# nii-yamagishilab/self-attention-tacotron

Hardware: AMD Instinct MI355X
Metric: mel-frames/sec (teacher-forced train step) (higher is better)
Workload: dtype bf16

## Files before the change

self-attention-tacotron_amd/csrc/flash.hip:

```cpp
#include <algorithm>
#include "common.h"

namespace {

constexpr int FHD = 128, FT = 64, FNT = 256;
constexpr float FLOG2E = 1.4426950408889634f;
typedef __attribute__((ext_vector_type(4))) unsigned int fu32x4_t;

__device__ __forceinline__ int kswz(int c) { return ((c & 3) << 1) ^ ((c >> 2) & 1); }

struct RowRegs { float4 v0[4], v1[4]; };
struct ColRegs { float4 v[2][4]; };
__device__ __forceinline__ void load_rows(const float* __restrict__ src, int64_t ld, int nvalid, int tid, RowRegs& R) {
#pragma unroll
  for (int g = 0; g < 4; ++g) {
    const int e = tid + FNT * g, row = min(e >> 4, nvalid - 1), chunk = e & 15;
    const float4* p = reinterpret_cast<const float4*>(src + (int64_t)row * ld + chunk * 8);
    R.v0[g] = p[0]; R.v1[g] = p[1];
  }
}
__device__ __forceinline__ void store_rows(const RowRegs& R, int nvalid, uint16_t* __restrict__ dst, int tid) {
#pragma unroll
  for (int g = 0; g < 4; ++g) {
    const int e = tid + FNT * g, row = e >> 4, chunk = e & 15;
    fu32x4_t w;
    w[0] = pack_bf16x2(R.v0[g].x, R.v0[g].y); w[1] = pack_bf16x2(R.v0[g].z, R.v0[g].w);
    w[2] = pack_bf16x2(R.v1[g].x, R.v1[g].y); w[3] = pack_bf16x2(R.v1[g].z, R.v1[g].w);
    if (row >= nvalid) w = (fu32x4_t){0u, 0u, 0u, 0u};
    *reinterpret_cast<fu32x4_t*>(dst + (chunk * FT + (row ^ kswz(chunk & 7))) * 8) = w;
  }
}
__device__ __forceinline__ void load_cols(const float* __restrict__ src, int64_t ld, int nvalid, int tid, ColRegs& R) {
  const int cq = tid & 31;
#pragma unroll
  for (int pass = 0; pass < 2; ++pass) {
    const int rq = (tid >> 5) + 8 * pass;
#pragma unroll
    for (int r = 0; r < 4; ++r)
      R.v[pass][r] = *reinterpret_cast<const float4*>(src + (int64_t)min(4 * rq + r, nvalid - 1) * ld + 4 * cq);
  }
}
__device__ __forceinline__ void store_cols(const ColRegs& R, int nvalid, uint16_t* __restrict__ dst, int tid) {
  const int cq = tid & 31;
  const int pc0 = (cq >> 4) * 64 + (cq & 15);
#pragma unroll
  for (int pass = 0; pass < 2; ++pass) {
    const int rq = (tid >> 5) + 8 * pass;
    const int ks = rq >> 3, q8 = rq & 7, eh = q8 >> 2, g = q8 & 3;
    float f[16];
#pragma unroll
    for (int r = 0; r < 4; ++r) {
      const bool ok = 4 * rq + r < nvalid;
      const float4 v = R.v[pass][r];
      f[4 * r] = ok ? v.x : 0.f; f[4 * r + 1] = ok ? v.y : 0.f; f[4 * r + 2] = ok ? v.z : 0.f; f[4 * r + 3] = ok ? v.w : 0.f;
    }
#pragma unroll
    for (int ii = 0; ii < 4; ++ii) {
      uint2 w;
      w.x = pack_bf16x2(f[ii], f[4 + ii]); w.y = pack_bf16x2(f[8 + ii], f[12 + ii]);
      *reinterpret_cast<uint2*>(dst + (((ks * 4 + g) * FHD + pc0 + 16 * ii) * 8) + 4 * eh) = w;
    }
  }
}
__device__ __forceinline__ bf16x8_t frag_rows(const uint16_t* img, int t, int ks, int lane) {
  const int chunk = 4 * ks + (lane >> 4), row = 16 * t + (lane & 15);
  return *reinterpret_cast<const bf16x8_t*>(img + (chunk * FT + (row ^ kswz(chunk & 7))) * 8);
}
__device__ __forceinline__ bf16x8_t frag_cols(const uint16_t* img, int n, int ks, int lane) {
  return *reinterpret_cast<const bf16x8_t*>(img + ((ks * 4 + (lane >> 4)) * FHD + 16 * n + (lane & 15)) * 8);
}
__device__ __forceinline__ bf16x8_t frag_global(const float* __restrict__ rowp, bool valid, int ks, int lane) {
  const float4* p = reinterpret_cast<const float4*>(rowp + 32 * ks + 8 * (lane >> 4));
  const float4 v0 = p[0], v1 = p[1];
  fu32x4_t w;
  w[0] = pack_bf16x2(v0.x, v0.y); w[1] = pack_bf16x2(v0.z, v0.w);
  w[2] = pack_bf16x2(v1.x, v1.y); w[3] = pack_bf16x2(v1.z, v1.w);
  if (!valid) w = (fu32x4_t){0u, 0u, 0u, 0u};
  return __builtin_bit_cast(bf16x8_t, w);
}
__device__ __forceinline__ bf16x8_t pack_b(const f32x4_t& lo, const f32x4_t& hi) {
  fu32x4_t w;
  w[0] = pack_bf16x2(lo[0], lo[1]); w[1] = pack_bf16x2(lo[2], lo[3]);
  w[2] = pack_bf16x2(hi[0], hi[1]); w[3] = pack_bf16x2(hi[2], hi[3]);
  return __builtin_bit_cast(bf16x8_t, w);
}
__device__ __forceinline__ float col_max(float v, int lane) {
  v = fmaxf(v, swz_xor(v, 16));
  return fmaxf(v, __int_as_float(__builtin_amdgcn_ds_bpermute((lane ^ 32) << 2, __float_as_int(v))));
}
__device__ __forceinline__ float col_sum(float v, int lane) {
  v += swz_xor(v, 16);
  return v + __int_as_float(__builtin_amdgcn_ds_bpermute((lane ^ 32) << 2, __float_as_int(v)));
}
__device__ __forceinline__ int unperm(int pr) { return (pr & ~63) | ((pr & 15) << 2) | ((pr & 63) >> 4); }

struct RowRegsB { fu32x4_t v[4]; };
struct ColRegsB { uint2 v[2][4]; };
__device__ __forceinline__ void load_rows(const uint16_t* __restrict__ src, int64_t ld, int nvalid, int tid, RowRegsB& R) {
#pragma unroll
  for (int g = 0; g < 4; ++g) {
    const int e = tid + FNT * g, row = min(e >> 4, nvalid - 1), chunk = e & 15;
    R.v[g] = *reinterpret_cast<const fu32x4_t*>(src + (int64_t)row * ld + chunk * 8);
  }
}
__device__ __forceinline__ void store_rows(const RowRegsB& R, int nvalid, uint16_t* __restrict__ dst, int tid) {
#pragma unroll
  for (int g = 0; g < 4; ++g) {
    const int e = tid + FNT * g, row = e >> 4, chunk = e & 15;
    fu32x4_t w = R.v[g];
    if (row >= nvalid) w = (fu32x4_t){0u, 0u, 0u, 0u};
    *reinterpret_cast<fu32x4_t*>(dst + (chunk * FT + (row ^ kswz(chunk & 7))) * 8) = w;
  }
}
__device__ __forceinline__ void load_cols(const uint16_t* __restrict__ src, int64_t ld, int nvalid, int tid, ColRegsB& R) {
  const int cq = tid & 31;
#pragma unroll
  for (int pass = 0; pass < 2; ++pass) {
    const int rq = (tid >> 5) + 8 * pass;
#pragma unroll
    for (int r = 0; r < 4; ++r)
      R.v[pass][r] = *reinterpret_cast<const uint2*>(src + (int64_t)min(4 * rq + r, nvalid - 1) * ld + 4 * cq);
  }
}
__device__ __forceinline__ void store_cols(const ColRegsB& R, int nvalid, uint16_t* __restrict__ dst, int tid) {
  const int cq = tid & 31;
  const int pc0 = (cq >> 4) * 64 + (cq & 15);
#pragma unroll
  for (int pass = 0; pass < 2; ++pass) {
    const int rq = (tid >> 5) + 8 * pass;
    const int ks = rq >> 3, q8 = rq & 7, eh = q8 >> 2, g = q8 & 3;
    uint32_t lo[4], hi[4];
#pragma unroll
    for (int r = 0; r < 4; ++r) {
      const bool ok = 4 * rq + r < nvalid;
      lo[r] = ok ? R.v[pass][r].x : 0u; hi[r] = ok ? R.v[pass][r].y : 0u;
    }
#pragma unroll
    for (int ii = 0; ii < 4; ++ii) {
      const uint32_t* w4 = (ii >> 1) ? hi : lo;
      uint2 w;
      if (ii & 1) { w.x = (w4[0] >> 16) | (w4[1] & 0xFFFF0000u); w.y = (w4[2] >> 16) | (w4[3] & 0xFFFF0000u); }
      else { w.x = (w4[0] & 0xFFFFu) | (w4[1] << 16); w.y = (w4[2] & 0xFFFFu) | (w4[3] << 16); }
      *reinterpret_cast<uint2*>(dst + (((ks * 4 + g) * FHD + pc0 + 16 * ii) * 8) + 4 * eh) = w;
    }
  }
}
__device__ __forceinline__ bf16x8_t frag_global(const uint16_t* __restrict__ rowp, bool valid, int ks, int lane) {
  fu32x4_t w = *reinterpret_cast<const fu32x4_t*>(rowp + 32 * ks + 8 * (lane >> 4));
  if (!valid) w = (fu32x4_t){0u, 0u, 0u, 0u};
  return __builtin_bit_cast(bf16x8_t, w);
}
template <bool BF> struct FSrc { typedef float T; typedef RowRegs Row; typedef ColRegs Col; };
template <> struct FSrc<true> { typedef uint16_t T; typedef RowRegsB Row; typedef ColRegsB Col; };

struct FlashArgs {
  const float* k; const float* v; const float* q; int64_t ld;
  float* o; int64_t ldo; float* lse;
  const float* dout; const float* delta;
  float* dk; float* dv; float* dq; int64_t ldd;
  int T, H, B; float scale; int causal;
  const uint16_t* kb; const uint16_t* vb; const uint16_t* qb; int64_t ldb;
  const uint16_t* doutb; int64_t ldob;
  uint16_t* kb_out; uint16_t* vb_out; uint16_t* qb_out;
  int tile_lo, tile_n;
  uint32_t thresh; float dscale; uint32_t stream; const uint32_t* seed;
};

__device__ __forceinline__ void flash_block(int nt, int BH, int& tile, int& bh, int lin = (int)blockIdx.x) {
  if ((BH & 7) == 0) { const int slot = lin >> 3; bh = (slot / nt) * 8 + (lin & 7); tile = slot - (slot / nt) * nt; }
  else { bh = lin / nt; tile = lin - bh * nt; }
}

template <bool DROP>
__attribute__((amdgpu_waves_per_eu(2, 2)))
__global__ __launch_bounds__(FNT) void flash_fwd_k(const FlashArgs a) {
  __shared__ __attribute__((aligned(16))) uint16_t lds[2 * FT * FHD];
  uint16_t* Ks = lds;
  uint16_t* Vt = lds + FT * FHD;
  const int tid = threadIdx.x, lane = tid & 63, wave = tid >> 6, g = lane >> 4;
  const int T = a.T, nqt = (T + FT - 1) / FT;
  int bx, bh; flash_block(nqt, a.B * a.H, bx, bh);
  const int b = bh / a.H, h = bh - b * a.H;
  const int qt = nqt - 1 - bx, i0 = qt * FT;
  const float* K = a.k + (int64_t)b * T * a.ld + h * FHD;
  const float* V = a.v + (int64_t)b * T * a.ld + h * FHD;
  const float* Q = a.q + (int64_t)b * T * a.ld + h * FHD;
  const int iq = i0 + 16 * wave + (lane & 15);
  bf16x8_t qb[4];
#pragma unroll
  for (int ks = 0; ks < 4; ++ks) qb[ks] = frag_global(Q + (int64_t)min(iq, T - 1) * a.ld, iq < T, ks, lane);
  if (a.qb_out && iq < T) {
    uint16_t* qo = a.qb_out + ((int64_t)b * T + iq) * a.ldb + h * FHD;
#pragma unroll
    for (int ks = 0; ks < 4; ++ks) *reinterpret_cast<bf16x8_t*>(qo + 32 * ks + 8 * g) = qb[ks];
  }
  const uint32_t seed = (a.thresh && a.seed) ? *a.seed : 0u;
  const float c2 = a.scale * FLOG2E;
  float m = -INFINITY, lsum = 0.f;
  f32x4_t oacc[8];
#pragma unroll
  for (int n = 0; n < 8; ++n) oacc[n] = (f32x4_t){0.f, 0.f, 0.f, 0.f};
  const int nkt = a.causal ? qt + 1 : nqt;
  RowRegs rk; ColRegs rv;
  load_rows(K, a.ld, T, tid, rk);
  load_cols(V, a.ld, T, tid, rv);
  for (int kt = 0; kt < nkt; ++kt) {
    const int j0 = kt * FT;
    lds_barrier();
    store_rows(rk, T - j0, Ks, tid);
    store_cols(rv, T - j0, Vt, tid);
    if (a.kb_out && kt == qt) {
#pragma unroll
      for (int gq = 0; gq < 4; ++gq) {
        const int e = tid + FNT * gq, row = e >> 4, chunk = e & 15;
        if (j0 + row < T) {
          fu32x4_t w;
          w[0] = pack_bf16x2(rk.v0[gq].x, rk.v0[gq].y); w[1] = pack_bf16x2(rk.v0[gq].z, rk.v0[gq].w);
          w[2] = pack_bf16x2(rk.v1[gq].x, rk.v1[gq].y); w[3] = pack_bf16x2(rk.v1[gq].z, rk.v1[gq].w);
          *reinterpret_cast<fu32x4_t*>(a.kb_out + ((int64_t)b * T + j0 + row) * a.ldb + h * FHD + chunk * 8) = w;
        }
      }
      const int cq = tid & 31;
#pragma unroll
      for (int pass = 0; pass < 2; ++pass)
#pragma unroll
        for (int r = 0; r < 4; ++r) {
          const int row = 4 * ((tid >> 5) + 8 * pass) + r;
          if (j0 + row < T) {
            const float4 v = rv.v[pass][r];
            uint2 w; w.x = pack_bf16x2(v.x, v.y); w.y = pack_bf16x2(v.z, v.w);
            *reinterpret_cast<uint2*>(a.vb_out + ((int64_t)b * T + j0 + row) * a.ldb + h * FHD + 4 * cq) = w;
          }
        }
    }
    if (kt + 1 < nkt) {
      load_rows(K + (int64_t)(j0 + FT) * a.ld, a.ld, T - j0 - FT, tid, rk);
      load_cols(V + (int64_t)(j0 + FT) * a.ld, a.ld, T - j0 - FT, tid, rv);
    }
    lds_barrier();
    f32x4_t s[4];
#pragma unroll
    for (int j = 0; j < 4; ++j) {
      s[j] = (f32x4_t){0.f, 0.f, 0.f, 0.f};
#pragma unroll
      for (int ks = 0; ks < 4; ++ks) s[j] = __builtin_amdgcn_mfma_f32_16x16x32_bf16(frag_rows(Ks, j, ks, lane), qb[ks], s[j], 0, 0, 0);
    }
    float mx = -INFINITY;
#pragma unroll
    for (int j = 0; j < 4; ++j)
#pragma unroll
      for (int r = 0; r < 4; ++r) {
        const int key = j0 + 16 * j + 4 * g + r;
        const bool ok = (key < T) & (!a.causal | (key <= iq));
        s[j][r] = ok ? s[j][r] * c2 : -INFINITY;
        mx = fmaxf(mx, s[j][r]);
      }
    mx = col_max(mx, lane);
    const float mn = fmaxf(m, mx);
    const float alpha = exp2f_(m - mn);
    float rs = 0.f;
#pragma unroll
    for (int j = 0; j < 4; ++j)
#pragma unroll
      for (int r = 0; r < 4; ++r) {
        const float pv = exp2f_(s[j][r] - mn);
        rs += pv;
        float pd = pv;
        if constexpr (DROP) {
          const int key = j0 + 16 * j + 4 * g + r;
          pd = satt_keep(seed, a.stream, (uint32_t)(((int64_t)bh * T + iq) * T + key), a.thresh) ? pv * a.dscale : 0.f;
        }
        s[j][r] = pd;
      }
    rs = col_sum(rs, lane);
    lsum = lsum * alpha + rs;
    m = mn;
#pragma unroll
    for (int n = 0; n < 8; ++n)
#pragma unroll
      for (int r = 0; r < 4; ++r) oacc[n][r] *= alpha;
#pragma unroll
    for (int ks = 0; ks < 2; ++ks) {
      const bf16x8_t pb = pack_b(s[2 * ks], s[2 * ks + 1]);
#pragma unroll
      for (int n = 0; n < 8; ++n) oacc[n] = __builtin_amdgcn_mfma_f32_16x16x32_bf16(frag_cols(Vt, n, ks, lane), pb, oacc[n], 0, 0, 0);
    }
  }
  if (iq < T) {
    const float inv = 1.f / lsum;
    float* orow = a.o + ((int64_t)b * T + iq) * a.ldo + h * FHD;
#pragma unroll
    for (int bq = 0; bq < 2; ++bq)
#pragma unroll
      for (int r = 0; r < 4; ++r) {
        const float4 v = make_float4(oacc[4 * bq][r] * inv, oacc[4 * bq + 1][r] * inv, oacc[4 * bq + 2][r] * inv, oacc[4 * bq + 3][r] * inv);
        *reinterpret_cast<float4*>(orow + 64 * bq + 16 * g + 4 * r) = v;
      }
    if (g == 0) a.lse[(int64_t)bh * T + iq] = m + log2f(lsum);
  }
}

__global__ __launch_bounds__(256) void flash_delta_k(const float* __restrict__ o, const float* __restrict__ dout, int64_t ldo,
                                                     float* __restrict__ delta, int B, int T, int H,
                                                     uint16_t* __restrict__ doutb, int64_t ldob, int r0, int r1) {
  const int lane = threadIdx.x & 63;
  const int64_t w = blockIdx.x * 4 + (threadIdx.x >> 6);
  const int nr = r1 - r0;
  if (w >= (int64_t)B * nr * H) return;
  const int64_t rr = w / H; const int h = (int)(w - rr * H);
  const int64_t row = (rr / nr) * T + r0 + (rr % nr);
  const float2 x = *reinterpret_cast<const float2*>(o + row * ldo + h * FHD + 2 * lane);
  const float2 y = *reinterpret_cast<const float2*>(dout + row * ldo + h * FHD + 2 * lane);
  if (doutb) *reinterpret_cast<uint32_t*>(doutb + row * ldob + h * FHD + 2 * lane) = pack_bf16x2(y.x, y.y);
  const float s = wave_sum(x.x * y.x + x.y * y.y);
  if (lane == 0) { const int64_t b = row / T; delta[(b * H + h) * T + (row - b * T)] = s; }
}

constexpr int DKV_LDS = (4 * FT * FHD) * 2 + 2 * FT * 4;
template <bool BF, bool DROP>
__device__ __forceinline__ void flash_dkv_body(const FlashArgs& a, uint16_t* dyn, int lin) {
  typedef typename FSrc<BF>::T ST;
  const int64_t sld = BF ? a.ldb : a.ld, dld = BF ? a.ldob : a.ldo;
  uint16_t* Qs = dyn; uint16_t* Qt = dyn + FT * FHD; uint16_t* Ds = dyn + 2 * FT * FHD; uint16_t* Dt = dyn + 3 * FT * FHD;
  float* Ls = reinterpret_cast<float*>(dyn + 4 * FT * FHD); float* dl = Ls + FT;
  const int tid = threadIdx.x, lane = tid & 63, wave = tid >> 6, g = lane >> 4;
  const int T = a.T, nt = (T + FT - 1) / FT;
  int kt, bh; flash_block(a.tile_n, a.B * a.H, kt, bh, lin);
  kt += a.tile_lo;
  const int b = bh / a.H, h = bh - b * a.H;
  const int j0 = kt * FT;
  const ST* K = (BF ? (const ST*)a.kb : (const ST*)a.k) + (int64_t)b * T * sld + h * FHD;
  const ST* V = (BF ? (const ST*)a.vb : (const ST*)a.v) + (int64_t)b * T * sld + h * FHD;
  const ST* Q = (BF ? (const ST*)a.qb : (const ST*)a.q) + (int64_t)b * T * sld + h * FHD;
  const ST* DO = (BF ? (const ST*)a.doutb : (const ST*)a.dout) + (int64_t)b * T * dld + h * FHD;
  const int key = j0 + 16 * wave + (lane & 15);
  bf16x8_t kb[4], vb[4];
#pragma unroll
  for (int ks = 0; ks < 4; ++ks) {
    kb[ks] = frag_global(K + (int64_t)min(key, T - 1) * sld, key < T, ks, lane);
    vb[ks] = frag_global(V + (int64_t)min(key, T - 1) * sld, key < T, ks, lane);
  }
  const uint32_t seed = (a.thresh && a.seed) ? *a.seed : 0u;
  const float c2 = a.scale * FLOG2E;
  f32x4_t dvt[8], dkt[8];
#pragma unroll
  for (int n = 0; n < 8; ++n) { dvt[n] = (f32x4_t){0.f, 0.f, 0.f, 0.f}; dkt[n] = dvt[n]; }
  struct Stage { typename FSrc<BF>::Row rq, rd; typename FSrc<BF>::Col cq, cd; float rl, rdl; };
  constexpr int NS = BF ? 2 : 1;
  Stage st[NS];
  auto request = [&](Stage& S, int i0) {
    load_rows(Q + (int64_t)i0 * sld, sld, T - i0, tid, S.rq);
    load_cols(Q + (int64_t)i0 * sld, sld, T - i0, tid, S.cq);
    load_rows(DO + (int64_t)i0 * dld, dld, T - i0, tid, S.rd);
    load_cols(DO + (int64_t)i0 * dld, dld, T - i0, tid, S.cd);
    const int64_t li = (int64_t)bh * T + min(i0 + (tid & (FT - 1)), T - 1);
    S.rl = a.lse[li]; S.rdl = a.delta[li];
  };
  const int qt0 = a.causal ? kt : 0;
  auto step = [&](Stage& S, int qt) {
    const int i0 = qt * FT;
    lds_barrier();
    store_rows(S.rq, T - i0, Qs, tid);
    store_cols(S.cq, T - i0, Qt, tid);
    store_rows(S.rd, T - i0, Ds, tid);
    store_cols(S.cd, T - i0, Dt, tid);
    if (tid < FT) {
      const bool ok = i0 + tid < T;
      Ls[tid] = ok ? S.rl : 0.f;
      dl[tid] = ok ? S.rdl : 0.f;
    }
    if (qt + NS < nt) request(S, i0 + NS * FT);
    lds_barrier();
    f32x4_t pd[4], ds[4];
#pragma unroll
    for (int i = 0; i < 4; ++i) {
      f32x4_t s = (f32x4_t){0.f, 0.f, 0.f, 0.f}, dp = s;
#pragma unroll
      for (int ks = 0; ks < 4; ++ks) {
        s = __builtin_amdgcn_mfma_f32_16x16x32_bf16(frag_rows(Qs, i, ks, lane), kb[ks], s, 0, 0, 0);
        dp = __builtin_amdgcn_mfma_f32_16x16x32_bf16(frag_rows(Ds, i, ks, lane), vb[ks], dp, 0, 0, 0);
      }
#pragma unroll
      for (int r = 0; r < 4; ++r) {
        const int ql = 16 * i + 4 * g + r, q = i0 + ql;
        const bool ok = (q < T) & (key < T) & (!a.causal | (key <= q));
        const float ev = exp2f_(s[r] * c2 - Ls[ql]);
        const float pv = ok ? ev : 0.f;
        if constexpr (DROP) {
          const bool keep = satt_keep(seed, a.stream, (uint32_t)(((int64_t)bh * T + q) * T + key), a.thresh);
          pd[i][r] = keep ? pv * a.dscale : 0.f;
          ds[i][r] = pv * ((keep ? dp[r] * a.dscale : 0.f) - dl[ql]);
        } else {
          pd[i][r] = pv;
          ds[i][r] = pv * (dp[r] - dl[ql]);
        }
      }
    }
#pragma unroll
    for (int ks = 0; ks < 2; ++ks) {
      const bf16x8_t pb = pack_b(pd[2 * ks], pd[2 * ks + 1]), sb = pack_b(ds[2 * ks], ds[2 * ks + 1]);
#pragma unroll
      for (int n = 0; n < 8; ++n) {
        dvt[n] = __builtin_amdgcn_mfma_f32_16x16x32_bf16(frag_cols(Dt, n, ks, lane), pb, dvt[n], 0, 0, 0);
        dkt[n] = __builtin_amdgcn_mfma_f32_16x16x32_bf16(frag_cols(Qt, n, ks, lane), sb, dkt[n], 0, 0, 0);
      }
    }
  };
  request(st[0], qt0 * FT);
  if (NS == 2 && qt0 + 1 < nt) request(st[NS - 1], (qt0 + 1) * FT);
  for (int qt = qt0; qt < nt; qt += NS) {
    step(st[0], qt);
    if (NS == 2 && qt + 1 < nt) step(st[NS - 1], qt + 1);
  }
  if (key < T) {
    float* dkr = a.dk + ((int64_t)b * T + key) * a.ldd + h * FHD;
    float* dvr = a.dv + ((int64_t)b * T + key) * a.ldd + h * FHD;
#pragma unroll
    for (int bq = 0; bq < 2; ++bq)
#pragma unroll
      for (int r = 0; r < 4; ++r) {
        const int col = 64 * bq + 16 * g + 4 * r;
        *reinterpret_cast<float4*>(dvr + col) = make_float4(dvt[4 * bq][r], dvt[4 * bq + 1][r], dvt[4 * bq + 2][r], dvt[4 * bq + 3][r]);
        *reinterpret_cast<float4*>(dkr + col) = make_float4(dkt[4 * bq][r] * a.scale, dkt[4 * bq + 1][r] * a.scale,
                                                             dkt[4 * bq + 2][r] * a.scale, dkt[4 * bq + 3][r] * a.scale);
      }
  }
}

template <bool BF, bool DROP>
__device__ __forceinline__ void flash_dq_body(const FlashArgs& a, uint16_t* lds, int lin) {
  typedef typename FSrc<BF>::T ST;
  const int64_t sld = BF ? a.ldb : a.ld, dld = BF ? a.ldob : a.ldo;
  uint16_t* Ks = lds; uint16_t* Kt = lds + FT * FHD; uint16_t* Vs = lds + 2 * FT * FHD;
  const int tid = threadIdx.x, lane = tid & 63, wave = tid >> 6, g = lane >> 4;
  const int T = a.T;
  int bx, bh; flash_block(a.tile_n, a.B * a.H, bx, bh, lin);
  const int b = bh / a.H, h = bh - b * a.H;
  const int qt = a.tile_lo + a.tile_n - 1 - bx, i0 = qt * FT;
  const ST* K = (BF ? (const ST*)a.kb : (const ST*)a.k) + (int64_t)b * T * sld + h * FHD;
  const ST* V = (BF ? (const ST*)a.vb : (const ST*)a.v) + (int64_t)b * T * sld + h * FHD;
  const ST* Q = (BF ? (const ST*)a.qb : (const ST*)a.q) + (int64_t)b * T * sld + h * FHD;
  const ST* DO = (BF ? (const ST*)a.doutb : (const ST*)a.dout) + (int64_t)b * T * dld + h * FHD;
  const int iq = i0 + 16 * wave + (lane & 15);
  bf16x8_t qb[4], dob[4];
#pragma unroll
  for (int ks = 0; ks < 4; ++ks) {
    qb[ks] = frag_global(Q + (int64_t)min(iq, T - 1) * sld, iq < T, ks, lane);
    dob[ks] = frag_global(DO + (int64_t)min(iq, T - 1) * dld, iq < T, ks, lane);
  }
  const float Lq_ = a.lse[(int64_t)bh * T + min(iq, T - 1)], dqr_ = a.delta[(int64_t)bh * T + min(iq, T - 1)];
  const float Lq = iq < T ? Lq_ : 0.f, dq_ = iq < T ? dqr_ : 0.f;
  const uint32_t seed = (a.thresh && a.seed) ? *a.seed : 0u;
  const float c2 = a.scale * FLOG2E;
  f32x4_t dqt[8];
#pragma unroll
  for (int n = 0; n < 8; ++n) dqt[n] = (f32x4_t){0.f, 0.f, 0.f, 0.f};
  const int nkt = a.causal ? qt + 1 : (T + FT - 1) / FT;
  struct Stage { typename FSrc<BF>::Row rk, rv; typename FSrc<BF>::Col ck; };
  constexpr int NS = BF ? 2 : 1;
  Stage st[NS];
  auto request = [&](Stage& S, int j0) {
    load_rows(K + (int64_t)j0 * sld, sld, T - j0, tid, S.rk);
    load_cols(K + (int64_t)j0 * sld, sld, T - j0, tid, S.ck);
    load_rows(V + (int64_t)j0 * sld, sld, T - j0, tid, S.rv);
  };
  auto step = [&](Stage& S, int kt) {
    const int j0 = kt * FT;
    lds_barrier();
    store_rows(S.rk, T - j0, Ks, tid);
    store_cols(S.ck, T - j0, Kt, tid);
    store_rows(S.rv, T - j0, Vs, tid);
    if (kt + NS < nkt) request(S, j0 + NS * FT);
    lds_barrier();
    f32x4_t ds[4];
#pragma unroll
    for (int j = 0; j < 4; ++j) {
      f32x4_t s = (f32x4_t){0.f, 0.f, 0.f, 0.f}, dp = s;
#pragma unroll
      for (int ks = 0; ks < 4; ++ks) {
        s = __builtin_amdgcn_mfma_f32_16x16x32_bf16(frag_rows(Ks, j, ks, lane), qb[ks], s, 0, 0, 0);
        dp = __builtin_amdgcn_mfma_f32_16x16x32_bf16(frag_rows(Vs, j, ks, lane), dob[ks], dp, 0, 0, 0);
      }
#pragma unroll
      for (int r = 0; r < 4; ++r) {
        const int key = j0 + 16 * j + 4 * g + r;
        const bool ok = (iq < T) & (key < T) & (!a.causal | (key <= iq));
        const float ev = exp2f_(s[r] * c2 - Lq);
        const float pv = ok ? ev : 0.f;
        float dpr = dp[r];
        if constexpr (DROP)
          dpr = satt_keep(seed, a.stream, (uint32_t)(((int64_t)bh * T + iq) * T + key), a.thresh) ? dpr * a.dscale : 0.f;
        ds[j][r] = pv * (dpr - dq_);
      }
    }
#pragma unroll
    for (int ks = 0; ks < 2; ++ks) {
      const bf16x8_t sb = pack_b(ds[2 * ks], ds[2 * ks + 1]);
#pragma unroll
      for (int n = 0; n < 8; ++n) dqt[n] = __builtin_amdgcn_mfma_f32_16x16x32_bf16(frag_cols(Kt, n, ks, lane), sb, dqt[n], 0, 0, 0);
    }
  };
  request(st[0], 0);
  if (NS == 2 && 1 < nkt) request(st[NS - 1], FT);
  for (int kt = 0; kt < nkt; kt += NS) {
    step(st[0], kt);
    if (NS == 2 && kt + 1 < nkt) step(st[NS - 1], kt + 1);
  }
  if (iq < T) {
    float* dqr = a.dq + ((int64_t)b * T + iq) * a.ldd + h * FHD;
#pragma unroll
    for (int bq = 0; bq < 2; ++bq)
#pragma unroll
      for (int r = 0; r < 4; ++r)
        *reinterpret_cast<float4*>(dqr + 64 * bq + 16 * g + 4 * r) =
            make_float4(dqt[4 * bq][r] * a.scale, dqt[4 * bq + 1][r] * a.scale, dqt[4 * bq + 2][r] * a.scale, dqt[4 * bq + 3][r] * a.scale);
  }
}

inline bool fl16(const void* p) { return (reinterpret_cast<uintptr_t>(p) & 15) == 0; }

}

template <bool BF, bool DROP>
__global__ __launch_bounds__(FNT) void flash_bwd_k(const FlashArgs a, const int ntiles) {
  extern __shared__ __attribute__((aligned(16))) uint16_t dyn[];
  const int lin = (int)blockIdx.x;
  if (lin < ntiles) flash_dkv_body<BF, DROP>(a, dyn, lin);
  else flash_dq_body<BF, DROP>(a, dyn, lin - ntiles);
}

static int flash_fwd_launch(const float* k, const float* v, const float* q, int64_t ld, float* o, int64_t ldo, float* lse,
                            int B, int T, int H, int head_dim, float scale, int causal, uint32_t drop_thresh,
                            float drop_scale, uint32_t drop_stream, const uint32_t* seed, uint16_t* kb, uint16_t* vb,
                            uint16_t* qb, int64_t ldb, void* stream) {
  if (!k || !v || !q || !o || !lse || B <= 0 || T <= 0 || H <= 0) return SATT_E_BADARG;
  if (head_dim != FHD) return SATT_E_UNSUPPORTED;
  if (ld % 4 || ldo % 4 || !fl16(k) || !fl16(v) || !fl16(q) || !fl16(o)) return SATT_E_UNSUPPORTED;
  if ((int64_t)B * H > 65535 || (int64_t)B * H * T * T >= (1ll << 32)) return SATT_E_UNSUPPORTED;
  if (kb && (!vb || !qb || ldb % 8 || !fl16(kb) || !fl16(vb) || !fl16(qb))) return SATT_E_BADARG;
  FlashArgs a{};
  a.k = k; a.v = v; a.q = q; a.ld = ld; a.o = o; a.ldo = ldo; a.lse = lse; a.T = T; a.H = H; a.B = B; a.scale = scale; a.causal = causal;
  a.thresh = drop_thresh; a.dscale = drop_scale; a.stream = drop_stream; a.seed = seed;
  a.kb_out = kb; a.vb_out = vb; a.qb_out = qb; a.ldb = ldb;
  if (drop_thresh) hipLaunchKernelGGL(flash_fwd_k<true>, dim3(((T + FT - 1) / FT) * B * H), dim3(FNT), 0, (hipStream_t)stream, a);
  else hipLaunchKernelGGL(flash_fwd_k<false>, dim3(((T + FT - 1) / FT) * B * H), dim3(FNT), 0, (hipStream_t)stream, a);
  SATT_LAUNCH_CHECK();
  return SATT_OK;
}

extern "C" int satt_flash_attn_fwd(const float* k, const float* v, const float* q, int64_t ld, float* o, int64_t ldo, float* lse,
                                   int B, int T, int H, int head_dim, float scale, int causal, uint32_t drop_thresh,
                                   float drop_scale, uint32_t drop_stream, const uint32_t* seed, void* stream) {
  return flash_fwd_launch(k, v, q, ld, o, ldo, lse, B, T, H, head_dim, scale, causal, drop_thresh, drop_scale, drop_stream, seed,
                          nullptr, nullptr, nullptr, 0, stream);
}

extern "C" int satt_flash_attn_fwd_b(const float* k, const float* v, const float* q, int64_t ld, float* o, int64_t ldo, float* lse,
                                     int B, int T, int H, int head_dim, float scale, int causal, uint32_t drop_thresh,
                                     float drop_scale, uint32_t drop_stream, const uint32_t* seed, uint16_t* kb, uint16_t* vb,
                                     uint16_t* qb, int64_t ldb, void* stream) {
  if (!kb) return SATT_E_BADARG;
  return flash_fwd_launch(k, v, q, ld, o, ldo, lse, B, T, H, head_dim, scale, causal, drop_thresh, drop_scale, drop_stream, seed,
                          kb, vb, qb, ldb, stream);
}

static int flash_bwd_launch(const float* k, const float* v, const float* q, int64_t ld, const float* o, const float* dout,
                            int64_t ldo, const float* lse, float* delta, float* dk, float* dv, float* dq, int64_t ldd,
                            int B, int T, int H, int head_dim, float scale, int causal, uint32_t drop_thresh,
                            float drop_scale, uint32_t drop_stream, const uint32_t* seed, int tile_lo, int tile_hi,
                            int with_delta, const uint16_t* kb, const uint16_t* vb, const uint16_t* qb, int64_t ldb,
                            uint16_t* doutb, int64_t ldob, void* stream) {
  const bool bf = kb != nullptr;
  if ((!bf && (!k || !v || !q)) || !o || !dout || !lse || !delta || !dk || !dv || !dq || B <= 0 || T <= 0 || H <= 0) return SATT_E_BADARG;
  if (head_dim != FHD) return SATT_E_UNSUPPORTED;
  if (ldo % 4 || ldd % 4 || !fl16(o) || !fl16(dout) || !fl16(dk) || !fl16(dv) || !fl16(dq)) return SATT_E_UNSUPPORTED;
  if (!bf && (ld % 4 || !fl16(k) || !fl16(v) || !fl16(q))) return SATT_E_UNSUPPORTED;
  if (bf && (!vb || !qb || !doutb || ldb % 8 || ldob % 8 || !fl16(kb) || !fl16(vb) || !fl16(qb) || !fl16(doutb))) return SATT_E_BADARG;
  if ((int64_t)B * H > 65535 || (int64_t)B * H * T * T >= (1ll << 32)) return SATT_E_UNSUPPORTED;
  const int nt = (T + FT - 1) / FT;
  if (tile_lo < 0 || tile_hi > nt || tile_lo >= tile_hi) return SATT_E_BADARG;
  if (!causal && (tile_lo != 0 || tile_hi != nt)) return SATT_E_BADARG;
  FlashArgs a{};
  a.k = k; a.v = v; a.q = q; a.ld = ld; a.ldo = ldo; a.lse = const_cast<float*>(lse); a.dout = dout; a.delta = delta;
  a.dk = dk; a.dv = dv; a.dq = dq; a.ldd = ldd; a.T = T; a.H = H; a.B = B; a.scale = scale; a.causal = causal;
  a.tile_lo = tile_lo; a.tile_n = tile_hi - tile_lo;
  a.thresh = drop_thresh; a.dscale = drop_scale; a.stream = drop_stream; a.seed = seed;
  a.kb = kb; a.vb = vb; a.qb = qb; a.ldb = ldb; a.doutb = doutb; a.ldob = ldob;
  hipStream_t s = (hipStream_t)stream;
  const int r0 = tile_lo * FT, r1 = std::min(tile_hi * FT, T);
  const int64_t nw = (int64_t)B * (r1 - r0) * H;
  if (with_delta)
    hipLaunchKernelGGL(flash_delta_k, dim3((unsigned)((nw + 3) / 4)), dim3(256), 0, s, o, dout, ldo, delta, B, T, H,
                       bf ? doutb : (uint16_t*)nullptr, ldob, r0, r1);
  static_assert(DKV_LDS >= 3 * FT * FHD * 2, "the dQ body fits the dK/dV body's LDS");
  const int ntiles = a.tile_n * B * H;
#define SATT_FLASH_BWD(BFV, DRV)                                                                                        \
  do {                                                                                                                    \
    (void)hipFuncSetAttribute((const void*)flash_bwd_k<BFV, DRV>, hipFuncAttributeMaxDynamicSharedMemorySize, DKV_LDS);   \
    hipLaunchKernelGGL((flash_bwd_k<BFV, DRV>), dim3(2 * ntiles), dim3(FNT), DKV_LDS, s, a, ntiles);                      \
  } while (0)
  if (bf) { if (drop_thresh) SATT_FLASH_BWD(true, true); else SATT_FLASH_BWD(true, false); }
  else { if (drop_thresh) SATT_FLASH_BWD(false, true); else SATT_FLASH_BWD(false, false); }
#undef SATT_FLASH_BWD
  SATT_LAUNCH_CHECK();
  return SATT_OK;
}

extern "C" int satt_flash_attn_bwd_tiles(const float* k, const float* v, const float* q, int64_t ld, const float* o, const float* dout,
                                         int64_t ldo, const float* lse, float* delta, float* dk, float* dv, float* dq, int64_t ldd,
                                         int B, int T, int H, int head_dim, float scale, int causal, uint32_t drop_thresh,
                                         float drop_scale, uint32_t drop_stream, const uint32_t* seed, int tile_lo, int tile_hi,
                                         int with_delta, void* stream) {
  return flash_bwd_launch(k, v, q, ld, o, dout, ldo, lse, delta, dk, dv, dq, ldd, B, T, H, head_dim, scale, causal, drop_thresh,
                          drop_scale, drop_stream, seed, tile_lo, tile_hi, with_delta, nullptr, nullptr, nullptr, 0, nullptr, 0, stream);
}

extern "C" int satt_flash_attn_bwd_tiles_b(const uint16_t* kb, const uint16_t* vb, const uint16_t* qb, int64_t ldb, const float* o,
                                           const float* dout, int64_t ldo, uint16_t* doutb, int64_t ldob, const float* lse,
                                           float* delta, float* dk, float* dv, float* dq, int64_t ldd, int B, int T, int H,
                                           int head_dim, float scale, int causal, uint32_t drop_thresh, float drop_scale,
                                           uint32_t drop_stream, const uint32_t* seed, int tile_lo, int tile_hi, int with_delta,
                                           void* stream) {
  if (!kb) return SATT_E_BADARG;
  return flash_bwd_launch(nullptr, nullptr, nullptr, 0, o, dout, ldo, lse, delta, dk, dv, dq, ldd, B, T, H, head_dim, scale, causal,
                          drop_thresh, drop_scale, drop_stream, seed, tile_lo, tile_hi, with_delta, kb, vb, qb, ldb, doutb, ldob, stream);
}

extern "C" int satt_flash_attn_bwd(const float* k, const float* v, const float* q, int64_t ld, const float* o, const float* dout,
                                   int64_t ldo, const float* lse, float* delta, float* dk, float* dv, float* dq, int64_t ldd,
                                   int B, int T, int H, int head_dim, float scale, int causal, uint32_t drop_thresh,
                                   float drop_scale, uint32_t drop_stream, const uint32_t* seed, void* stream) {
  return satt_flash_attn_bwd_tiles(k, v, q, ld, o, dout, ldo, lse, delta, dk, dv, dq, ldd, B, T, H, head_dim, scale, causal,
                                   drop_thresh, drop_scale, drop_stream, seed, 0, T > 0 ? (T + FT - 1) / FT : 0, 1, stream);
}
```

Measured before the change: 3.643 million.

## Use LDS transpose reads instead of storing transposed Q/dO/K tiles in flash backward

Drops the separate column-major (transposed) LDS copies of Q, dO and K in the backward kernels. The transposed MFMA operands are now read directly from the row-major tiles with ds_read_tr16_b64, using a new XOR swizzle. This halves LDS use and removes the duplicate global loads and transpose stores, and the bf16 double-buffer stage is dropped in favour of a single stage with waves_per_eu(2,2). The delta kernel is also rewritten so each wave handles two or four rows using float4 loads and DPP reductions, which loses some prefetch depth in exchange for higher occupancy.

```diff
diff --git a/self-attention-tacotron_amd/csrc/flash.hip b/self-attention-tacotron_amd/csrc/flash.hip
--- a/self-attention-tacotron_amd/csrc/flash.hip
+++ b/self-attention-tacotron_amd/csrc/flash.hip
@@ -7,7 +7,7 @@
 constexpr float FLOG2E = 1.4426950408889634f;
 typedef __attribute__((ext_vector_type(4))) unsigned int fu32x4_t;
 
-__device__ __forceinline__ int kswz(int c) { return ((c & 3) << 1) ^ ((c >> 2) & 1); }
+__device__ __forceinline__ int kswz(int c) { return ((c & 1) * 12) | ((c >> 1) & 3); }
 
 struct RowRegs { float4 v0[4], v1[4]; };
 struct ColRegs { float4 v[2][4]; };
@@ -68,6 +68,16 @@
 }
 __device__ __forceinline__ bf16x8_t frag_cols(const uint16_t* img, int n, int ks, int lane) {
   return *reinterpret_cast<const bf16x8_t*>(img + ((ks * 4 + (lane >> 4)) * FHD + 16 * n + (lane & 15)) * 8);
+}
+__device__ __forceinline__ bf16x8_t frag_tr(const uint16_t* img, int n, int ks, int lane) {
+  typedef __attribute__((ext_vector_type(4))) short s16x4_t;
+  typedef __attribute__((address_space(3))) s16x4_t* lds_s16x4_p;
+  const int g = lane >> 4, q = (lane >> 2) & 3, p = lane & 3;
+  const int chunk = 2 * n + (p >> 1), row = 32 * ks + 4 * g + q;
+  const uint16_t* p0 = img + (chunk * FT + (row ^ kswz(chunk & 7))) * 8 + 4 * (p & 1);
+  const s16x4_t lo = __builtin_amdgcn_ds_read_tr16_b64_v4i16((lds_s16x4_p)p0);
+  const s16x4_t hi = __builtin_amdgcn_ds_read_tr16_b64_v4i16((lds_s16x4_p)(p0 + 16 * 8));
+  return __builtin_shufflevector(lo, hi, 0, 1, 2, 3, 4, 5, 6, 7);
 }
 __device__ __forceinline__ bf16x8_t frag_global(const float* __restrict__ rowp, bool valid, int ks, int lane) {
   const float4* p = reinterpret_cast<const float4*>(rowp + 32 * ks + 8 * (lane >> 4));
@@ -95,7 +105,6 @@
 __device__ __forceinline__ int unperm(int pr) { return (pr & ~63) | ((pr & 15) << 2) | ((pr & 63) >> 4); }
 
 struct RowRegsB { fu32x4_t v[4]; };
-struct ColRegsB { uint2 v[2][4]; };
 __device__ __forceinline__ void load_rows(const uint16_t* __restrict__ src, int64_t ld, int nvalid, int tid, RowRegsB& R) {
 #pragma unroll
   for (int g = 0; g < 4; ++g) {
@@ -112,46 +121,13 @@
     *reinterpret_cast<fu32x4_t*>(dst + (chunk * FT + (row ^ kswz(chunk & 7))) * 8) = w;
   }
 }
-__device__ __forceinline__ void load_cols(const uint16_t* __restrict__ src, int64_t ld, int nvalid, int tid, ColRegsB& R) {
-  const int cq = tid & 31;
-#pragma unroll
-  for (int pass = 0; pass < 2; ++pass) {
-    const int rq = (tid >> 5) + 8 * pass;
-#pragma unroll
-    for (int r = 0; r < 4; ++r)
-      R.v[pass][r] = *reinterpret_cast<const uint2*>(src + (int64_t)min(4 * rq + r, nvalid - 1) * ld + 4 * cq);
-  }
-}
-__device__ __forceinline__ void store_cols(const ColRegsB& R, int nvalid, uint16_t* __restrict__ dst, int tid) {
-  const int cq = tid & 31;
-  const int pc0 = (cq >> 4) * 64 + (cq & 15);
-#pragma unroll
-  for (int pass = 0; pass < 2; ++pass) {
-    const int rq = (tid >> 5) + 8 * pass;
-    const int ks = rq >> 3, q8 = rq & 7, eh = q8 >> 2, g = q8 & 3;
-    uint32_t lo[4], hi[4];
-#pragma unroll
-    for (int r = 0; r < 4; ++r) {
-      const bool ok = 4 * rq + r < nvalid;
-      lo[r] = ok ? R.v[pass][r].x : 0u; hi[r] = ok ? R.v[pass][r].y : 0u;
-    }
-#pragma unroll
-    for (int ii = 0; ii < 4; ++ii) {
-      const uint32_t* w4 = (ii >> 1) ? hi : lo;
-      uint2 w;
-      if (ii & 1) { w.x = (w4[0] >> 16) | (w4[1] & 0xFFFF0000u); w.y = (w4[2] >> 16) | (w4[3] & 0xFFFF0000u); }
-      else { w.x = (w4[0] & 0xFFFFu) | (w4[1] << 16); w.y = (w4[2] & 0xFFFFu) | (w4[3] << 16); }
-      *reinterpret_cast<uint2*>(dst + (((ks * 4 + g) * FHD + pc0 + 16 * ii) * 8) + 4 * eh) = w;
-    }
-  }
-}
 __device__ __forceinline__ bf16x8_t frag_global(const uint16_t* __restrict__ rowp, bool valid, int ks, int lane) {
   fu32x4_t w = *reinterpret_cast<const fu32x4_t*>(rowp + 32 * ks + 8 * (lane >> 4));
   if (!valid) w = (fu32x4_t){0u, 0u, 0u, 0u};
   return __builtin_bit_cast(bf16x8_t, w);
 }
-template <bool BF> struct FSrc { typedef float T; typedef RowRegs Row; typedef ColRegs Col; };
-template <> struct FSrc<true> { typedef uint16_t T; typedef RowRegsB Row; typedef ColRegsB Col; };
+template <bool BF> struct FSrc { typedef float T; typedef RowRegs Row; };
+template <> struct FSrc<true> { typedef uint16_t T; typedef RowRegsB Row; };
 
 struct FlashArgs {
   const float* k; const float* v; const float* q; int64_t ld;
@@ -300,29 +276,51 @@
   }
 }
 
+template <int NP>
 __global__ __launch_bounds__(256) void flash_delta_k(const float* __restrict__ o, const float* __restrict__ dout, int64_t ldo,
                                                      float* __restrict__ delta, int B, int T, int H,
                                                      uint16_t* __restrict__ doutb, int64_t ldob, int r0, int r1) {
-  const int lane = threadIdx.x & 63;
-  const int64_t w = blockIdx.x * 4 + (threadIdx.x >> 6);
-  const int nr = r1 - r0;
-  if (w >= (int64_t)B * nr * H) return;
-  const int64_t rr = w / H; const int h = (int)(w - rr * H);
-  const int64_t row = (rr / nr) * T + r0 + (rr % nr);
-  const float2 x = *reinterpret_cast<const float2*>(o + row * ldo + h * FHD + 2 * lane);
-  const float2 y = *reinterpret_cast<const float2*>(dout + row * ldo + h * FHD + 2 * lane);
-  if (doutb) *reinterpret_cast<uint32_t*>(doutb + row * ldob + h * FHD + 2 * lane) = pack_bf16x2(y.x, y.y);
-  const float s = wave_sum(x.x * y.x + x.y * y.y);
-  if (lane == 0) { const int64_t b = row / T; delta[(b * H + h) * T + (row - b * T)] = s; }
-}
-
-constexpr int DKV_LDS = (4 * FT * FHD) * 2 + 2 * FT * 4;
+  const int lane = threadIdx.x & 63, half = lane >> 5, l32 = lane & 31;
+  const uint32_t nr = r1 - r0, n = (uint32_t)B * nr * H;
+  const uint32_t w0 = (blockIdx.x * 4 + (threadIdx.x >> 6)) * 2 * NP;
+  if (w0 >= n) return;
+  float4 x[NP], y[NP]; int64_t row[NP]; int hh[NP]; bool ok[NP];
+#pragma unroll
+  for (int k = 0; k < NP; ++k) {
+    const uint32_t w = w0 + 2 * k + half;
+    ok[k] = w < n;
+    const uint32_t wc = min(w, n - 1), rr = wc / (uint32_t)H, bb = rr / nr;
+    hh[k] = (int)(wc - rr * H);
+    row[k] = (int64_t)bb * T + r0 + (rr - bb * nr);
+    x[k] = *reinterpret_cast<const float4*>(o + row[k] * ldo + hh[k] * FHD + 4 * l32);
+    y[k] = *reinterpret_cast<const float4*>(dout + row[k] * ldo + hh[k] * FHD + 4 * l32);
+  }
+#pragma unroll
+  for (int k = 0; k < NP; ++k) {
+    if (doutb && ok[k]) {
+      uint2 wv; wv.x = pack_bf16x2(y[k].x, y[k].y); wv.y = pack_bf16x2(y[k].z, y[k].w);
+      *reinterpret_cast<uint2*>(doutb + row[k] * ldob + hh[k] * FHD + 4 * l32) = wv;
+    }
+    float q = __fmaf_rn(x[k].x, y[k].x, __fmul_rn(x[k].y, y[k].y)) + __fmaf_rn(x[k].z, y[k].z, __fmul_rn(x[k].w, y[k].w));
+    SATT_DPP_ADD(q, 0xB1);
+    SATT_DPP_ADD(q, 0x4E);
+    SATT_DPP_ADD(q, 0x141);
+    SATT_DPP_ADD(q, 0x140);
+    const float sa = __int_as_float(__builtin_amdgcn_readlane(__float_as_int(q), 0)) +
+                     __int_as_float(__builtin_amdgcn_readlane(__float_as_int(q), 16));
+    const float sb = __int_as_float(__builtin_amdgcn_readlane(__float_as_int(q), 32)) +
+                     __int_as_float(__builtin_amdgcn_readlane(__float_as_int(q), 48));
+    if (l32 == 0 && ok[k]) { const int64_t b = row[k] / T; delta[(b * H + hh[k]) * T + (row[k] - b * T)] = half ? sb : sa; }
+  }
+}
+
+constexpr int DKV_LDS = (2 * FT * FHD) * 2 + 2 * FT * 4;
 template <bool BF, bool DROP>
 __device__ __forceinline__ void flash_dkv_body(const FlashArgs& a, uint16_t* dyn, int lin) {
   typedef typename FSrc<BF>::T ST;
   const int64_t sld = BF ? a.ldb : a.ld, dld = BF ? a.ldob : a.ldo;
-  uint16_t* Qs = dyn; uint16_t* Qt = dyn + FT * FHD; uint16_t* Ds = dyn + 2 * FT * FHD; uint16_t* Dt = dyn + 3 * FT * FHD;
-  float* Ls = reinterpret_cast<float*>(dyn + 4 * FT * FHD); float* dl = Ls + FT;
+  uint16_t* Qs = dyn; uint16_t* Ds = dyn + FT * FHD;
+  float* Ls = reinterpret_cast<float*>(dyn + 2 * FT * FHD); float* dl = Ls + FT;
   const int tid = threadIdx.x, lane = tid & 63, wave = tid >> 6, g = lane >> 4;
   const int T = a.T, nt = (T + FT - 1) / FT;
   int kt, bh; flash_block(a.tile_n, a.B * a.H, kt, bh, lin);
@@ -345,14 +343,11 @@
   f32x4_t dvt[8], dkt[8];
 #pragma unroll
   for (int n = 0; n < 8; ++n) { dvt[n] = (f32x4_t){0.f, 0.f, 0.f, 0.f}; dkt[n] = dvt[n]; }
-  struct Stage { typename FSrc<BF>::Row rq, rd; typename FSrc<BF>::Col cq, cd; float rl, rdl; };
-  constexpr int NS = BF ? 2 : 1;
-  Stage st[NS];
+  struct Stage { typename FSrc<BF>::Row rq, rd; float rl, rdl; };
+  Stage st;
   auto request = [&](Stage& S, int i0) {
     load_rows(Q + (int64_t)i0 * sld, sld, T - i0, tid, S.rq);
-    load_cols(Q + (int64_t)i0 * sld, sld, T - i0, tid, S.cq);
     load_rows(DO + (int64_t)i0 * dld, dld, T - i0, tid, S.rd);
-    load_cols(DO + (int64_t)i0 * dld, dld, T - i0, tid, S.cd);
     const int64_t li = (int64_t)bh * T + min(i0 + (tid & (FT - 1)), T - 1);
     S.rl = a.lse[li]; S.rdl = a.delta[li];
   };
@@ -361,15 +356,13 @@
     const int i0 = qt * FT;
     lds_barrier();
     store_rows(S.rq, T - i0, Qs, tid);
-    store_cols(S.cq, T - i0, Qt, tid);
     store_rows(S.rd, T - i0, Ds, tid);
-    store_cols(S.cd, T - i0, Dt, tid);
     if (tid < FT) {
       const bool ok = i0 + tid < T;
       Ls[tid] = ok ? S.rl : 0.f;
       dl[tid] = ok ? S.rdl : 0.f;
     }
-    if (qt + NS < nt) request(S, i0 + NS * FT);
+    if (qt + 1 < nt) request(S, i0 + FT);
     lds_barrier();
     f32x4_t pd[4], ds[4];
 #pragma unroll
@@ -401,29 +394,22 @@
       const bf16x8_t pb = pack_b(pd[2 * ks], pd[2 * ks + 1]), sb = pack_b(ds[2 * ks], ds[2 * ks + 1]);
 #pragma unroll
       for (int n = 0; n < 8; ++n) {
-        dvt[n] = __builtin_amdgcn_mfma_f32_16x16x32_bf16(frag_cols(Dt, n, ks, lane), pb, dvt[n], 0, 0, 0);
-        dkt[n] = __builtin_amdgcn_mfma_f32_16x16x32_bf16(frag_cols(Qt, n, ks, lane), sb, dkt[n], 0, 0, 0);
+        dvt[n] = __builtin_amdgcn_mfma_f32_16x16x32_bf16(frag_tr(Ds, n, ks, lane), pb, dvt[n], 0, 0, 0);
+        dkt[n] = __builtin_amdgcn_mfma_f32_16x16x32_bf16(frag_tr(Qs, n, ks, lane), sb, dkt[n], 0, 0, 0);
       }
     }
   };
-  request(st[0], qt0 * FT);
-  if (NS == 2 && qt0 + 1 < nt) request(st[NS - 1], (qt0 + 1) * FT);
-  for (int qt = qt0; qt < nt; qt += NS) {
-    step(st[0], qt);
-    if (NS == 2 && qt + 1 < nt) step(st[NS - 1], qt + 1);
-  }
+  request(st, qt0 * FT);
+  for (int qt = qt0; qt < nt; ++qt) step(st, qt);
   if (key < T) {
     float* dkr = a.dk + ((int64_t)b * T + key) * a.ldd + h * FHD;
     float* dvr = a.dv + ((int64_t)b * T + key) * a.ldd + h * FHD;
 #pragma unroll
-    for (int bq = 0; bq < 2; ++bq)
-#pragma unroll
-      for (int r = 0; r < 4; ++r) {
-        const int col = 64 * bq + 16 * g + 4 * r;
-        *reinterpret_cast<float4*>(dvr + col) = make_float4(dvt[4 * bq][r], dvt[4 * bq + 1][r], dvt[4 * bq + 2][r], dvt[4 * bq + 3][r]);
-        *reinterpret_cast<float4*>(dkr + col) = make_float4(dkt[4 * bq][r] * a.scale, dkt[4 * bq + 1][r] * a.scale,
-                                                             dkt[4 * bq + 2][r] * a.scale, dkt[4 * bq + 3][r] * a.scale);
-      }
+    for (int n = 0; n < 8; ++n) {
+      const int col = 16 * n + 4 * g;
+      *reinterpret_cast<float4*>(dvr + col) = make_float4(dvt[n][0], dvt[n][1], dvt[n][2], dvt[n][3]);
+      *reinterpret_cast<float4*>(dkr + col) = make_float4(dkt[n][0] * a.scale, dkt[n][1] * a.scale, dkt[n][2] * a.scale, dkt[n][3] * a.scale);
+    }
   }
 }
 
@@ -431,7 +417,7 @@
 __device__ __forceinline__ void flash_dq_body(const FlashArgs& a, uint16_t* lds, int lin) {
   typedef typename FSrc<BF>::T ST;
   const int64_t sld = BF ? a.ldb : a.ld, dld = BF ? a.ldob : a.ldo;
-  uint16_t* Ks = lds; uint16_t* Kt = lds + FT * FHD; uint16_t* Vs = lds + 2 * FT * FHD;
+  uint16_t* Ks = lds; uint16_t* Vs = lds + FT * FHD;
   const int tid = threadIdx.x, lane = tid & 63, wave = tid >> 6, g = lane >> 4;
   const int T = a.T;
   int bx, bh; flash_block(a.tile_n, a.B * a.H, bx, bh, lin);
@@ -456,21 +442,18 @@
 #pragma unroll
   for (int n = 0; n < 8; ++n) dqt[n] = (f32x4_t){0.f, 0.f, 0.f, 0.f};
   const int nkt = a.causal ? qt + 1 : (T + FT - 1) / FT;
-  struct Stage { typename FSrc<BF>::Row rk, rv; typename FSrc<BF>::Col ck; };
-  constexpr int NS = BF ? 2 : 1;
-  Stage st[NS];
+  struct Stage { typename FSrc<BF>::Row rk, rv; };
+  Stage st;
   auto request = [&](Stage& S, int j0) {
     load_rows(K + (int64_t)j0 * sld, sld, T - j0, tid, S.rk);
-    load_cols(K + (int64_t)j0 * sld, sld, T - j0, tid, S.ck);
     load_rows(V + (int64_t)j0 * sld, sld, T - j0, tid, S.rv);
   };
   auto step = [&](Stage& S, int kt) {
     const int j0 = kt * FT;
     lds_barrier();
     store_rows(S.rk, T - j0, Ks, tid);
-    store_cols(S.ck, T - j0, Kt, tid);
     store_rows(S.rv, T - j0, Vs, tid);
-    if (kt + NS < nkt) request(S, j0 + NS * FT);
+    if (kt + 1 < nkt) request(S, j0 + FT);
     lds_barrier();
     f32x4_t ds[4];
 #pragma unroll
@@ -497,23 +480,17 @@
     for (int ks = 0; ks < 2; ++ks) {
       const bf16x8_t sb = pack_b(ds[2 * ks], ds[2 * ks + 1]);
 #pragma unroll
-      for (int n = 0; n < 8; ++n) dqt[n] = __builtin_amdgcn_mfma_f32_16x16x32_bf16(frag_cols(Kt, n, ks, lane), sb, dqt[n], 0, 0, 0);
+      for (int n = 0; n < 8; ++n) dqt[n] = __builtin_amdgcn_mfma_f32_16x16x32_bf16(frag_tr(Ks, n, ks, lane), sb, dqt[n], 0, 0, 0);
     }
   };
-  request(st[0], 0);
-  if (NS == 2 && 1 < nkt) request(st[NS - 1], FT);
-  for (int kt = 0; kt < nkt; kt += NS) {
-    step(st[0], kt);
-    if (NS == 2 && kt + 1 < nkt) step(st[NS - 1], kt + 1);
-  }
+  request(st, 0);
+  for (int kt = 0; kt < nkt; ++kt) step(st, kt);
   if (iq < T) {
     float* dqr = a.dq + ((int64_t)b * T + iq) * a.ldd + h * FHD;
 #pragma unroll
-    for (int bq = 0; bq < 2; ++bq)
-#pragma unroll
-      for (int r = 0; r < 4; ++r)
-        *reinterpret_cast<float4*>(dqr + 64 * bq + 16 * g + 4 * r) =
-            make_float4(dqt[4 * bq][r] * a.scale, dqt[4 * bq + 1][r] * a.scale, dqt[4 * bq + 2][r] * a.scale, dqt[4 * bq + 3][r] * a.scale);
+    for (int n = 0; n < 8; ++n)
+      *reinterpret_cast<float4*>(dqr + 16 * n + 4 * g) =
+          make_float4(dqt[n][0] * a.scale, dqt[n][1] * a.scale, dqt[n][2] * a.scale, dqt[n][3] * a.scale);
   }
 }
 
@@ -522,6 +499,7 @@
 }
 
 template <bool BF, bool DROP>
+__attribute__((amdgpu_waves_per_eu(2, 2)))
 __global__ __launch_bounds__(FNT) void flash_bwd_k(const FlashArgs a, const int ntiles) {
   extern __shared__ __attribute__((aligned(16))) uint16_t dyn[];
   const int lin = (int)blockIdx.x;
@@ -589,10 +567,12 @@
   hipStream_t s = (hipStream_t)stream;
   const int r0 = tile_lo * FT, r1 = std::min(tile_hi * FT, T);
   const int64_t nw = (int64_t)B * (r1 - r0) * H;
-  if (with_delta)
-    hipLaunchKernelGGL(flash_delta_k, dim3((unsigned)((nw + 3) / 4)), dim3(256), 0, s, o, dout, ldo, delta, B, T, H,
-                       bf ? doutb : (uint16_t*)nullptr, ldob, r0, r1);
-  static_assert(DKV_LDS >= 3 * FT * FHD * 2, "the dQ body fits the dK/dV body's LDS");
+  if (with_delta) {
+    uint16_t* db = bf ? doutb : (uint16_t*)nullptr;
+    if (nw >= 16384) hipLaunchKernelGGL(flash_delta_k<2>, dim3((unsigned)((nw + 15) / 16)), dim3(256), 0, s, o, dout, ldo, delta, B, T, H, db, ldob, r0, r1);
+    else hipLaunchKernelGGL(flash_delta_k<1>, dim3((unsigned)((nw + 7) / 8)), dim3(256), 0, s, o, dout, ldo, delta, B, T, H, db, ldob, r0, r1);
+  }
+  static_assert(DKV_LDS >= 2 * FT * FHD * 2, "the dQ body fits the dK/dV body's LDS");
   const int ntiles = a.tile_n * B * H;
 #define SATT_FLASH_BWD(BFV, DRV)                                                                                        \
   do {                                                                                                                    \
```

New measurement: 3.652 million, median of 6. Within noise of the previous version (+0.2%).
